# yli421/koopman-mpc-portfolio-rebalancing

Measured on AMD Instinct MI355X. Metric: MPC window-solves/sec (batched backtest) at 1/2/4/8 MI355X vs host-CPU ref, higher is better.
Workload: dtype f32 rollout (fp32 GEMMs as three exact bf16 planes); mixed f32->f64 IPM solve (float32 phase to mu 3e-5, float64 finish: stopping rule, status and W in float64); 1 GPU; C3 (BASELINE configs[2]): 65536 windows/GPU, 100 assets, latent 256, H=10, obs 2000, GenericKM enc [1024,1024], L1-turnover MPC c=1e-3 tau=0.2 no-short; windows_per_gpu=65536, parallelism=1 GPU, no collective

## Files before the change

include/kmpc.h:

```cpp
#ifndef KMPC_H
#define KMPC_H

#include <stddef.h>

#ifdef __cplusplus
extern "C" {
#endif

#define KMPC_OK               0
#define KMPC_ERR_INVALID     -1
#define KMPC_ERR_UNSUPPORTED -2
#define KMPC_ERR_WORKSPACE   -3
#define KMPC_ERR_LAUNCH      -4

#define KMPC_STATUS_OPTIMAL            0
#define KMPC_STATUS_OPTIMAL_INACCURATE 1
#define KMPC_STATUS_INFEASIBLE         2
#define KMPC_STATUS_UNBOUNDED          3
#define KMPC_STATUS_SOLVER_ERROR       4

#define KMPC_MAX_H 21
#define KMPC_MAX_N 1024

#define KMPC_PATH_AUTO     0
// ... 2 lines not shown
#define KMPC_PATH_LARGE    2
#define KMPC_PATH_REGISTER_UNPACKED 3
#define KMPC_PRECISION_AUTO  0
#define KMPC_PRECISION_F64   1
#define KMPC_PRECISION_MIXED 2
#define KMPC_MIXED_MIN_B 2048
typedef struct kmpc_solve_desc {
    int    B;
    int    N;
    int    H;
    double cost_coeff;
    double max_turnover;
    int    allow_short;
    int    max_iter;
    double tol;
    int    return_full_W;
    int    n_refine;
    int    path;
    int    precision;
    double mu_handoff;
} kmpc_solve_desc;

int kmpc_solve(const kmpc_solve_desc* desc,
               const float*  yhat,
               const double* w_prev,
               double*       w_out,
               int*          status,
               double*       obj,
               int*          iters,
               void* workspace, size_t ws_bytes, void* stream);

int kmpc_solve_box(const kmpc_solve_desc* desc, double max_weight,
                   const float*  yhat,
                   const double* w_prev,
                   double*       w_out,
                   int*          status,
                   double*       obj,
                   int*          iters,
                   void* stream);

int kmpc_gross_returns(size_t n, const float* yhat, float* R, void* stream);

#define KMPC_MODEL_GENERIC 0
#define KMPC_MODEL_LISTA   1
#define KMPC_ACT_RELU 0
#define KMPC_ACT_TANH 1
#define KMPC_ACT_GELU 2
#define KMPC_NORM_ID   0
#define KMPC_NORM_BALL 1
#define KMPC_MAX_LAYERS 8
#define KMPC_DTYPE_F32  0
#define KMPC_DTYPE_BF16 1
#define KMPC_DTYPE_F32_F32MFMA 2
typedef struct kmpc_mlp {
    int n_layers;
    int dims[KMPC_MAX_LAYERS + 1];
    int act;
    int last_relu;
    const float* weight[KMPC_MAX_LAYERS];
    const float* bias[KMPC_MAX_LAYERS];
} kmpc_mlp;

#define KMPC_LATENT_AUTO       0
#define KMPC_LATENT_UNFUSED    1
#define KMPC_LATENT_SEQUENTIAL 2

typedef struct kmpc_rollout_desc {
    int B;
    int N;
    int H;
    int L;
    int obs;
    int model_kind;
    int norm_fn;
    kmpc_mlp encoder;
    const float* lista_S;
    int   lista_loops;
    float lista_thresh;
    const float* kmat;
    kmpc_mlp decoder;
    const float* mean;
    const float* std;
    int obs_ld;
    int dtype;
    int latent_unfused;
} kmpc_rollout_desc;

int kmpc_rollout(const kmpc_rollout_desc* desc,
                 const float* obs,
                 float*       yhat,
                 void* workspace, size_t ws_bytes, void* stream);

int kmpc_standardize(int T, int N, const double* log_returns, const double* mean, const double* std,
                     float* z, void* stream);

int kmpc_window(const kmpc_rollout_desc* rdesc, const kmpc_solve_desc* sdesc,
                const float*  obs,
                const double* w_prev,
                float*        yhat,
                double*       w_out, int* status, double* obj, int* iters,
                void* workspace, size_t ws_bytes, void* stream);

typedef struct kmpc_backtest_desc {
    int    P;
    int    N;
    int    S;
// ... 79 lines not shown
```

koopman_mpc_portfolio_rebalancing_amd/_lib.py:

```python
from __future__ import annotations

import ctypes
import os

import torch

_HERE = os.path.dirname(os.path.abspath(__file__))
LIB_PATH = os.path.join(_HERE, "libkmpc.so")

KMPC_OK = 0
KMPC_ERR_UNSUPPORTED = -2
KMPC_MAX_LAYERS = 8
KMPC_MAX_N = 1024
KMPC_MAX_H = 21

MODEL_GENERIC, MODEL_LISTA = 0, 1
ACT = {"relu": 0, "tanh": 1, "gelu": 2}
NORM = {"id": 0, "ball": 1}
DTYPE = {"fp32": 0, "bf16": 1, "fp32_f32mfma": 2}
LATENT_FORM = {"auto": 0, "unfused": 1, "sequential": 2}

STATUS_NAMES = {0: "optimal", 1: "optimal_inaccurate", 2: "infeasible", 3: "unbounded",
                4: "solver_error"}

KMPC_MV_MAX_HN = 1024
KMPC_MV_MAX_H = 16

EXPORTED_SYMBOLS = ("kmpc_solve", "kmpc_rollout", "kmpc_window", "kmpc_workspace_bytes",
                    "kmpc_backtest_step", "kmpc_backtest_metrics", "kmpc_standardize", "kmpc_strerror",
                    "kmpc_version", "kmpc_solve_mv", "kmpc_rolling_moments", "kmpc_solve_mv_ws",
                    "kmpc_mv_workspace_bytes", "kmpc_gross_returns", "kmpc_backtest_run",
                    "kmpc_backtest_sweep", "kmpc_solve_box", "kmpc_solve_mv_box",
                    "kmpc_rolling_moments_paths", "kmpc_markowitz_run", "kmpc_markowitz_sweep")

PATH_AUTO, PATH_REGISTER, PATH_LARGE, PATH_REGISTER_UNPACKED = 0, 1, 2, 3
PRECISION_AUTO, PRECISION_F64, PRECISION_MIXED = 0, 1, 2
MIXED_MIN_B = 2048
PACK_MIN_B = 512

ABI_VERSION = "0.7.0"


class KmpcError(RuntimeError):
    pass


class SolveDesc(ctypes.Structure):
    _fields_ = [("B", ctypes.c_int), ("N", ctypes.c_int), ("H", ctypes.c_int),
                ("cost_coeff", ctypes.c_double), ("max_turnover", ctypes.c_double),
                ("allow_short", ctypes.c_int), ("max_iter", ctypes.c_int),
                ("tol", ctypes.c_double), ("return_full_W", ctypes.c_int), ("n_refine", ctypes.c_int),
                ("path", ctypes.c_int), ("precision", ctypes.c_int), ("mu_handoff", ctypes.c_double)]


class MvDesc(ctypes.Structure):
    _fields_ = [("B", ctypes.c_int), ("N", ctypes.c_int), ("H", ctypes.c_int),
                ("gamma", ctypes.c_double), ("cost_coeff", ctypes.c_double),
                ("allow_short", ctypes.c_int), ("max_iter", ctypes.c_int),
                ("tol", ctypes.c_double), ("return_full_W", ctypes.c_int)]


class Mlp(ctypes.Structure):
    _fields_ = [("n_layers", ctypes.c_int), ("dims", ctypes.c_int * (KMPC_MAX_LAYERS + 1)),
                ("act", ctypes.c_int), ("last_relu", ctypes.c_int),
                ("weight", ctypes.c_void_p * KMPC_MAX_LAYERS),
                ("bias", ctypes.c_void_p * KMPC_MAX_LAYERS)]


class RolloutDesc(ctypes.Structure):
    _fields_ = [("B", ctypes.c_int), ("N", ctypes.c_int), ("H", ctypes.c_int), ("L", ctypes.c_int),
                ("obs", ctypes.c_int), ("model_kind", ctypes.c_int), ("norm_fn", ctypes.c_int),
                ("encoder", Mlp), ("lista_S", ctypes.c_void_p), ("lista_loops", ctypes.c_int),
# ... 120 lines not shown
```

koopman_mpc_portfolio_rebalancing_amd/csrc/kmpc_rollout.hip:

```cpp
#include <hip/hip_runtime.h>
#include <math.h>
#include <stdint.h>

#include "kmpc_internal.h"

namespace kmpc {

typedef float f32x16 __attribute__((ext_vector_type(16)));
typedef float f32x4 __attribute__((ext_vector_type(4)));
typedef __bf16 bf16x8 __attribute__((ext_vector_type(8)));
typedef __bf16 bf16x4 __attribute__((ext_vector_type(4)));

enum Epi : int {
    EPI_NONE = 0,
    EPI_ACT = 1,
    EPI_SHRINK = 2,
    EPI_DESTD = 3,
};

struct GemmArgs {
    int M, N, K;
    const float* A; int lda;
    const float* B; int ldb;
    const float* bias;
// ... 433 lines not shown
                    c = __builtin_amdgcn_mfma_f32_32x32x16_bf16(af[0][a], bf[1][b], c, 0, 0, 0);
                    c = __builtin_amdgcn_mfma_f32_32x32x16_bf16(af[0][a], bf[0][b], c, 0, 0, 0);
                    acc[a][b] = c;
                }
        }
    };
    if constexpr (DB) {
        fetch(kbeg);
        stage(0);
        if (kbeg + BKT < kend) fetch(kbeg + BKT);
        __syncthreads();
        int buf = 0;
        for (int k0 = kbeg; k0 < kend; k0 += BKT) {
            substep(buf, 0);
            if (k0 + BKT < kend) {
                stage(buf ^ 1);
                if (k0 + 2 * BKT < kend) fetch(k0 + 2 * BKT);
            }
#pragma unroll
            for (int st = 1; st < NS; ++st) substep(buf, st);
            __syncthreads();
            buf ^= 1;
        }
    } else {
        fetch(kbeg);
        for (int k0 = kbeg; k0 < kend; k0 += BKT) {
            stage(0);
            __syncthreads();
            if (k0 + BKT < kend) fetch(k0 + BKT);
#pragma unroll
            for (int st = 0; st < NS; ++st) substep(0, st);
            __syncthreads();
        }
    }
    if (g.ksplit > 1) {
        float* P = g.part + (size_t)blockIdx.z * g.M * g.N;
#pragma unroll
        for (int a = 0; a < WM; ++a)
#pragma unroll
            for (int b = 0; b < WN; ++b) {
                const int n = n0 + wn + b * 32 + (lane & 31);
                if (n >= g.N) continue;
#pragma unroll
                for (int r = 0; r < 16; ++r) {
                    const int m = m0 + wm + a * 32 + (r & 3) + 8 * (r >> 2) + 4 * (lane >> 5);
                    if (m < g.M) P[(size_t)m * g.N + n] = acc[a][b][r];
                }
            }
        return;
    }
    epilogue<WM, WN>(g, acc, m0, n0, wm, wn, lane);
}

__global__ void shrink_kernel(const float* x, float* y, size_t n, float thr) {
    const size_t i = (size_t)blockIdx.x * blockDim.x + threadIdx.x;
    if (i < n) {
        const float v = x[i];
        const float av = fabsf(v) - thr;
        y[i] = (av > 0.0f) ? copysignf(av, v) : 0.0f * v;
    }
}

__global__ void ball_norm_kernel(float* x, int M, int L) {
    const int row = blockIdx.x * (blockDim.x / 64) + threadIdx.x / 64, lane = threadIdx.x & 63;
    if (row >= M) return;
    float* p = x + (size_t)row * L;
    float s = 0.0f;
    for (int j = lane; j < L; j += 64) s += p[j] * p[j];
#pragma unroll
    for (int o = 32; o >= 1; o >>= 1) s += __shfl_xor(s, o, 64);
    const float nrm = sqrtf(s);
    for (int j = lane; j < L; j += 64) p[j] = p[j] / nrm;
}

__global__ void transpose_kernel(const float* in, float* out, int R, int Cc) {
    __shared__ float tile[32][33];
    const int bx = blockIdx.x * 32, by = blockIdx.y * 32;
    const int tx = threadIdx.x & 31, ty = threadIdx.x >> 5;
    for (int r = ty; r < 32; r += 8) {
        const int i = by + r, j = bx + tx;
        if (i < R && j < Cc) tile[r][tx] = in[(size_t)i * Cc + j];
    }
    __syncthreads();
    for (int r = ty; r < 32; r += 8) {
        const int j = bx + r, i = by + tx;
        if (i < R && j < Cc) out[(size_t)j * R + i] = tile[tx][r];
    }
}

struct LatentArgs {
    int B, L, N, H;
    const float* z0;
    const float* zparts; int nparts; const float* zbias;
    const float* Kt;
    const float* K;
    const float* D;
    const float* bias;
    const float* mean; const float* stdv;
    float* yhat;
    int ball;
};
constexpr int LAT_ROWS = 32;

__device__ __forceinline__ float latent_z0(const LatentArgs& a, int m, int col) {
    const size_t i = (size_t)m * a.L + col;
    if (a.nparts == 0) return a.z0[i];
// ... 349 lines not shown
        __syncthreads();
    }
}

__global__ void tile_epilogue_kernel(int H, int N, const float* bias, const float* mean, const float* stdv,
                                     float* tb, float* tm, float* ts) {
    const int i = blockIdx.x * blockDim.x + threadIdx.x;
    if (i >= H * N) return;
    const int n = i % N;
    tb[i] = bias ? bias[n] : 0.0f;
    tm[i] = mean[n];
    ts[i] = stdv[n];
}

static bool latent_fusable(const kmpc_rollout_desc* d) {
    return d->latent_unfused != KMPC_LATENT_UNFUSED && d->dtype != KMPC_DTYPE_BF16 && d->decoder.n_layers == 1 && d->L % 32 == 0 &&
           d->L <= 512 && ((uintptr_t)d->decoder.weight[0] & 15) == 0 &&
           !(d->model_kind == KMPC_MODEL_GENERIC && d->norm_fn != KMPC_NORM_ID && d->norm_fn != KMPC_NORM_BALL);
}

#ifndef KMPC_F32_SPLITK
#define KMPC_F32_SPLITK 4
#endif
constexpr int SPLITK = KMPC_F32_SPLITK;
constexpr int SPLITK_BUF = 8;
constexpr size_t SPLITK_ELEMS = (size_t)256 * 64 * 64;

#ifndef KMPC_GEMM_MID
#define KMPC_GEMM_MID 44
#endif
#ifndef KMPC_BF16_SPLITK
#define KMPC_BF16_SPLITK 1
#endif
#ifndef KMPC_Z0_FUSE
#define KMPC_Z0_FUSE 1
#endif
#ifndef KMPC_BF16_SPLIT_MINK
#define KMPC_BF16_SPLIT_MINK 2048
#endif
#ifndef KMPC_BF16_SMALL
#define KMPC_BF16_SMALL 1
#endif
#ifndef KMPC_GEMM_BIG
#define KMPC_GEMM_BIG 42
#endif
template <int WM, int WN, int GM = 2, int GN = 2>
static void launch_f32(dim3 grid, hipStream_t s, const GemmArgs& g) {
    if (g.bf16 == 2)
        hipLaunchKernelGGL((gemm_nt_x3_kernel<WM, WN, GM, GN>), grid, dim3(64 * GM * GN), 0, s, g);
    else
        hipLaunchKernelGGL((gemm_nt_kernel<WM, WN, BK, GM, GN>), grid, dim3(64 * GM * GN), 0, s, g);
}

static int gemm(GemmArgs g, hipStream_t s, float* part = nullptr, int* nparts = nullptr) {
    if (nparts) *nparts = 0;
    if (g.M <= 0 || g.N <= 0) return KMPC_OK;
    g.ksplit = 1;
    dim3 grid((g.N + BN - 1) / BN, (g.M + BM - 1) / BM);
    if (g.bf16 == 1) {
        const bool few = (size_t)grid.x * grid.y < 256;
        if (KMPC_BF16_SPLITK && few && part && g.K >= KMPC_BF16_SPLIT_MINK && (size_t)g.M * g.N <= SPLITK_ELEMS) {
            g.ksplit = SPLITK_BUF;
            g.part = part;
            hipLaunchKernelGGL(gemm_nt_bf16_kernel<2>, dim3(grid.x, grid.y, SPLITK_BUF), dim3(256), 0, s, g);
            const size_t n = (size_t)g.M * g.N;
            hipLaunchKernelGGL(splitk_epilogue_kernel, dim3((unsigned)((n + 255) / 256)), dim3(256), 0, s, g);
            return hipGetLastError() == hipSuccess ? KMPC_OK : KMPC_ERR_LAUNCH;
        }
        if (few && KMPC_BF16_SMALL)
            hipLaunchKernelGGL(gemm_nt_bf16_kernel<1>, dim3((g.N + 63) / 64, (g.M + 63) / 64), dim3(256), 0, s, g);
        else
            hipLaunchKernelGGL(gemm_nt_bf16_kernel<2>, grid, dim3(256), 0, s, g);
    } else if ((size_t)grid.x * grid.y < 512) {
        dim3 grid64((g.N + 63) / 64, (g.M + 63) / 64);
        static_assert(SPLITK >= 2 && SPLITK <= SPLITK_BUF, "split-K slices");
        if (part && (size_t)grid64.x * grid64.y < 256 && g.K >= 128 * SPLITK) {
            g.ksplit = SPLITK;
            g.part = part;
            launch_f32<1, 1>(dim3(grid64.x, grid64.y, SPLITK), s, g);
            if (nparts && g.epi == EPI_NONE) {
                *nparts = SPLITK;
                return hipGetLastError() == hipSuccess ? KMPC_OK : KMPC_ERR_LAUNCH;
            }
            const size_t n = (size_t)g.M * g.N;
            hipLaunchKernelGGL(splitk_epilogue_kernel, dim3((unsigned)((n + 255) / 256)), dim3(256), 0, s, g);
            return hipGetLastError() == hipSuccess ? KMPC_OK : KMPC_ERR_LAUNCH;
        }
        if (KMPC_GEMM_MID == 21)
            launch_f32<2, 1>(dim3((g.N + 63) / 64, (g.M + 127) / 128), s, g);
        else if (KMPC_GEMM_MID == 12)
            launch_f32<1, 2>(dim3((g.N + 127) / 128, (g.M + 63) / 64), s, g);
        else if (KMPC_GEMM_MID == 22)
            launch_f32<2, 2>(grid, s, g);
        else if (KMPC_GEMM_MID == 42)
            launch_f32<1, 2, 4, 2>(grid, s, g);
        else if (KMPC_GEMM_MID == 44)
            launch_f32<1, 1, 4, 4>(grid, s, g);
        else
            launch_f32<1, 1>(grid64, s, g);
    } else if (KMPC_GEMM_BIG == 42) {
        launch_f32<1, 2, 4, 2>(grid, s, g);
    } else if (KMPC_GEMM_BIG == 44) {
        launch_f32<1, 1, 4, 4>(grid, s, g);
    } else if (KMPC_GEMM_BIG == 82) {
        launch_f32<1, 2, 8, 2>(dim3((g.N + 127) / 128, (g.M + 255) / 256), s, g);
    } else {
        launch_f32<2, 2>(grid, s, g);
    }
    return hipGetLastError() == hipSuccess ? KMPC_OK : KMPC_ERR_LAUNCH;
}

static GemmArgs linear(int M, int N, int K, const float* A, int lda, const float* W, const float* bias,
                       float* C, int ldc) {
    GemmArgs g = {};
    g.M = M; g.N = N; g.K = K; g.A = A; g.lda = lda; g.B = W; g.ldb = K; g.bias = bias;
    g.C = C; g.ldc = ldc; g.epi = EPI_NONE;
    return g;
}

static size_t align256(size_t x) { return (x + 255) & ~(size_t)255; }

static int max_width(const kmpc_mlp& m) {
    int w = 0;
    for (int l = 0; l <= m.n_layers; ++l) w = m.dims[l] > w ? m.dims[l] : w;
    return w;
}

size_t rollout_workspace_bytes(const kmpc_rollout_desc* d) {
    if (!d) return 0;
    const size_t B = (size_t)d->B;
    int wmax = d->L;
    const int we = max_width(d->encoder), wd = max_width(d->decoder);
    if (we > wmax) wmax = we;
    if (wd > wmax) wmax = wd;
    size_t bytes = 0;
    bytes += align256(sizeof(float) * (size_t)d->L * d->L);
    bytes += align256(sizeof(float) * (size_t)d->L * d->L);
    bytes += 2 * align256(sizeof(float) * B * wmax);
    bytes += 2 * align256(sizeof(float) * B * d->L);
    const size_t part = B * (size_t)wmax < SPLITK_ELEMS ? B * (size_t)wmax : SPLITK_ELEMS;
    bytes += align256(sizeof(float) * SPLITK_BUF * part);
    bytes += align256((size_t)6 * d->L * (d->L + 32 * (size_t)((d->N + 31) / 32)));
    bytes += align256(sizeof(float) * (size_t)d->H * d->N * (d->L + 3));
    return bytes;
}

static int run_mlp(const kmpc_mlp& m, int Bn, const float* X, int ldx, float* out, int ldo,
                   int last_cols, int last_epi, const float* mean, const float* stdv, float* ping,
                   float* pong, int wmax, int bf16, hipStream_t s, float* part, int* last_nparts = nullptr) {
    const float* cur = X;
    int ldc = ldx;
    for (int l = 0; l < m.n_layers; ++l) {
        const bool last = (l == m.n_layers - 1);
        const int nout = last ? last_cols : m.dims[l + 1];
        float* dst = last ? out : ((l & 1) ? pong : ping);
        GemmArgs g = linear(Bn, nout, m.dims[l], cur, ldc, m.weight[l], m.bias[l], dst,
                            last ? ldo : wmax);
        g.bf16 = bf16;
        if (!last) { g.epi = EPI_ACT; g.act = m.act; }
        else if (last_epi == EPI_DESTD) { g.epi = EPI_DESTD; g.mean = mean; g.stdv = stdv; }
        else if (m.last_relu) { g.epi = EPI_ACT; g.act = KMPC_ACT_RELU; }
        int rc = gemm(g, s, part, last ? last_nparts : nullptr);
        if (rc) return rc;
        cur = dst;
        ldc = wmax;
    }
    return KMPC_OK;
}

int rollout_launch(const kmpc_rollout_desc* d, const float* obs, float* yhat, void* ws,
                   size_t ws_bytes, hipStream_t s) {
    if (!d || !obs || !yhat || !d->kmat || !d->mean || !d->std) return KMPC_ERR_INVALID;
    if (d->B < 0 || d->N < 1 || d->H < 1 || d->L < 1 || d->obs < d->N) return KMPC_ERR_INVALID;
    if (d->encoder.n_layers < 1 || d->encoder.n_layers > KMPC_MAX_LAYERS) return KMPC_ERR_INVALID;
    if (d->decoder.n_layers < 1 || d->decoder.n_layers > KMPC_MAX_LAYERS) return KMPC_ERR_INVALID;
    if (d->encoder.dims[0] != d->obs || d->encoder.dims[d->encoder.n_layers] != d->L) return KMPC_ERR_INVALID;
    if (d->decoder.dims[0] != d->L || d->decoder.dims[d->decoder.n_layers] < d->N) return KMPC_ERR_INVALID;
    if (d->model_kind == KMPC_MODEL_LISTA && !d->lista_S) return KMPC_ERR_INVALID;
    if (ws_bytes < rollout_workspace_bytes(d) || (!ws && ws_bytes)) return KMPC_ERR_WORKSPACE;
    if (d->obs_ld < 0 || (d->obs_ld > 0 && d->obs_ld < d->N)) return KMPC_ERR_INVALID;
    if (d->dtype != KMPC_DTYPE_F32 && d->dtype != KMPC_DTYPE_BF16 && d->dtype != KMPC_DTYPE_F32_F32MFMA)
        return KMPC_ERR_INVALID;
    if (d->latent_unfused < KMPC_LATENT_AUTO || d->latent_unfused > KMPC_LATENT_SEQUENTIAL) return KMPC_ERR_INVALID;
    const int bf = d->dtype == KMPC_DTYPE_F32 ? KMPC_F32_GEMM : d->dtype == KMPC_DTYPE_BF16 ? 1 : 0;
    if (d->B == 0) return KMPC_OK;
    const int Bn = d->B, L = d->L, N = d->N, H = d->H;
    const int obs_ld = d->obs_ld > 0 ? d->obs_ld : d->obs;
    int wmax = L;
    {
        const int we = max_width(d->encoder), wd = max_width(d->decoder);
        if (we > wmax) wmax = we;
        if (wd > wmax) wmax = wd;
    }
    char* p = (char*)ws;
    float* Kt = (float*)p;   p += align256(sizeof(float) * (size_t)L * L);
    float* St = (float*)p;   p += align256(sizeof(float) * (size_t)L * L);
    float* ping = (float*)p; p += align256(sizeof(float) * (size_t)Bn * wmax);
    float* pong = (float*)p; p += align256(sizeof(float) * (size_t)Bn * wmax);
    float* z0 = (float*)p;   p += align256(sizeof(float) * (size_t)Bn * L);
    float* z1 = (float*)p;   p += align256(sizeof(float) * (size_t)Bn * L);
    float* part = (float*)p;
    {
        const size_t pe = (size_t)Bn * wmax < SPLITK_ELEMS ? (size_t)Bn * wmax : SPLITK_ELEMS;
        p += align256(sizeof(float) * SPLITK_BUF * pe);
    }
    __bf16* planes = (__bf16*)p;
    p += align256((size_t)6 * L * (L + 32 * (size_t)((N + 31) / 32)));
    float* Wpow = (float*)p;
    int rc;
    const bool latpow = KMPC_LATPOW && d->latent_unfused == KMPC_LATENT_AUTO && latent_fusable(d) && Bn >= KMPC_LATPOW_MINB &&
                        !(d->model_kind == KMPC_MODEL_GENERIC && d->norm_fn == KMPC_NORM_BALL);
    const bool lat16 = latent_fusable(d) && (Bn < KMPC_LAT16_MAXB || L <= 16 * KMPC_LAT16_WAVES);
    const bool kdir = lat16 && Bn < KMPC_LAT16_MAXB && !latpow;
    dim3 tg((L + 31) / 32, (L + 31) / 32);
    if (!kdir) hipLaunchKernelGGL(transpose_kernel, tg, dim3(256), 0, s, d->kmat, Kt, L, L);
    if (d->model_kind == KMPC_MODEL_LISTA)
        hipLaunchKernelGGL(transpose_kernel, tg, dim3(256), 0, s, d->lista_S, St, L, L);
    if (hipGetLastError() != hipSuccess) return KMPC_ERR_LAUNCH;

    int znparts = 0;
    const bool zfuse = KMPC_Z0_FUSE && d->model_kind == KMPC_MODEL_GENERIC && latent_fusable(d) &&
                       d->norm_fn != KMPC_NORM_BALL && !latpow;
    if (d->model_kind == KMPC_MODEL_GENERIC) {
        rc = run_mlp(d->encoder, Bn, obs, obs_ld, z0, L, L, EPI_NONE, nullptr, nullptr, ping, pong, wmax, bf, s, part,
                     zfuse ? &znparts : nullptr);
        if (rc) return rc;
        if (d->norm_fn == KMPC_NORM_BALL)
            hipLaunchKernelGGL(ball_norm_kernel, dim3((Bn + 3) / 4), dim3(256), 0, s, z0, Bn, L);
    } else {
        rc = run_mlp(d->encoder, Bn, obs, obs_ld, z1, L, L, EPI_NONE, nullptr, nullptr, ping, pong, wmax, bf, s, part);
        if (rc) return rc;
        const size_t n = (size_t)Bn * L;
        hipLaunchKernelGGL(shrink_kernel, dim3((unsigned)((n + 255) / 256)), dim3(256), 0, s, z1, z0, n,
                           d->lista_thresh);
        float* zc = z0;
        float* zn = ping;
        for (int it = 0; it < d->lista_loops; ++it) {
            GemmArgs g = linear(Bn, L, L, zc, L, St, nullptr, zn, L);
            g.epi = EPI_SHRINK; g.R = z1; g.ldr = L; g.thr = d->lista_thresh; g.bf16 = bf;
            if ((rc = gemm(g, s, part))) return rc;
            float* t = zc; zc = zn; zn = t;
        }
        if (zc != z0 && hipMemcpyAsync(z0, zc, sizeof(float) * n, hipMemcpyDeviceToDevice, s) != hipSuccess)
            return KMPC_ERR_LAUNCH;
    }
    if (hipGetLastError() != hipSuccess) return KMPC_ERR_LAUNCH;
    if (znparts > 0 && !latent_fusable(d)) return KMPC_ERR_INVALID;

    if (latpow) {
        const int HN = H * N;
        float* tb = Wpow + (size_t)HN * L;
        float* tm = tb + HN;
        float* ts = tm + HN;
        hipLaunchKernelGGL(latent_powers_kernel, dim3(N), dim3(64 * ((L + 63) / 64)), sizeof(double) * L, s,
                           d->decoder.weight[0], Kt, L, N, H, Wpow);
        hipLaunchKernelGGL(tile_epilogue_kernel, dim3((HN + 255) / 256), dim3(256), 0, s, H, N, d->decoder.bias[0],
                           d->mean, d->std, tb, tm, ts);
        GemmArgs g = linear(Bn, HN, L, z0, L, Wpow, tb, yhat, HN);
        g.epi = EPI_DESTD; g.mean = tm; g.stdv = ts; g.bf16 = bf;
        if ((rc = gemm(g, s, part))) return rc;
        return hipGetLastError() == hipSuccess ? KMPC_OK : KMPC_ERR_LAUNCH;
    }
    if (latent_fusable(d)) {
        LatentArgs la;
        la.B = Bn; la.L = L; la.N = N; la.H = H; la.z0 = z0; la.Kt = Kt; la.K = d->kmat; la.D = d->decoder.weight[0];
        la.zparts = part; la.nparts = znparts;
        la.zbias = d->encoder.bias[d->encoder.n_layers - 1];
        la.bias = d->decoder.bias[0]; la.mean = d->mean; la.stdv = d->std; la.yhat = yhat;
        la.ball = d->model_kind == KMPC_MODEL_GENERIC && d->norm_fn == KMPC_NORM_BALL;
        if (lat16) {
            const size_t lds = sizeof(float) * 2 * LAT16 * (L + 4);
            if (kdir)
                hipLaunchKernelGGL((latent_steps16_kernel<KMPC_LAT16_WAVES, true>), dim3((Bn + LAT16 - 1) / LAT16),
                                   dim3(64 * KMPC_LAT16_WAVES), lds, s, la);
            else
                hipLaunchKernelGGL((latent_steps16_kernel<KMPC_LAT16_WAVES, false>), dim3((Bn + LAT16 - 1) / LAT16),
                                   dim3(64 * KMPC_LAT16_WAVES), lds, s, la);
            return hipGetLastError() == hipSuccess ? KMPC_OK : KMPC_ERR_LAUNCH;
        }
        if (KMPC_LATX3 && bf == 2 && !la.ball && L == 256) {
            const int Dpad = 32 * ((N + 31) / 32);
            __bf16* Kp = planes;
            __bf16* Dp = planes + (size_t)3 * L * L;
            const size_t nk = (size_t)L * L, nd = (size_t)Dpad * L;
            hipLaunchKernelGGL(split_planes_kernel, dim3((unsigned)((nk + 255) / 256)), dim3(256), 0, s, Kt, L, L, L, L, Kp);
            hipLaunchKernelGGL(split_planes_kernel, dim3((unsigned)((nd + 255) / 256)), dim3(256), 0, s, la.D, N, Dpad, L,
                               L, Dp);
            const size_t lds = sizeof(__bf16) * 3 * LATX3_ROWS * (L + 8);
            hipLaunchKernelGGL((latent_steps_x3_kernel<8, 256>), dim3((Bn + LATX3_ROWS - 1) / LATX3_ROWS), dim3(512), lds,
                               s, la, (const __bf16*)Kp, (const __bf16*)Dp, Dpad);
            return hipGetLastError() == hipSuccess ? KMPC_OK : KMPC_ERR_LAUNCH;
        }
        const size_t lds = sizeof(float) * 2 * LAT_ROWS * (L + 4);
        hipLaunchKernelGGL(latent_steps_kernel<KMPC_LAT_WAVES>, dim3((Bn + LAT_ROWS - 1) / LAT_ROWS),
                           dim3(64 * KMPC_LAT_WAVES), lds, s, la);
        return hipGetLastError() == hipSuccess ? KMPC_OK : KMPC_ERR_LAUNCH;
    }
    float* zc = z0;
    float* zn = z1;
    for (int k = 0; k < H; ++k) {
        GemmArgs g = linear(Bn, L, L, zc, L, Kt, nullptr, zn, L);
        g.bf16 = bf;
        if ((rc = gemm(g, s, part))) return rc;
        if (d->model_kind == KMPC_MODEL_GENERIC && d->norm_fn == KMPC_NORM_BALL)
            hipLaunchKernelGGL(ball_norm_kernel, dim3((Bn + 3) / 4), dim3(256), 0, s, zn, Bn, L);
        rc = run_mlp(d->decoder, Bn, zn, L, yhat + (size_t)k * N, H * N, N, EPI_DESTD, d->mean, d->std,
                     ping, pong, wmax, bf, s, part);
        if (rc) return rc;
        float* t = zc; zc = zn; zn = t;
    }
    return hipGetLastError() == hipSuccess ? KMPC_OK : KMPC_ERR_LAUNCH;
}

__global__ void standardize_kernel(int T, int N, const double* y, const double* mean, const double* stdv,
                                   float* z) {
    const size_t i = (size_t)blockIdx.x * blockDim.x + threadIdx.x;
    if (i >= (size_t)T * N) return;
    const int n = (int)(i % N);
    z[i] = (float)((y[i] - mean[n]) / stdv[n]);
}

int standardize_launch(int T, int N, const double* y, const double* mean, const double* stdv, float* z,
                       hipStream_t s) {
    const size_t n = (size_t)T * N;
    if (n == 0) return KMPC_OK;
    hipLaunchKernelGGL(standardize_kernel, dim3((unsigned)((n + 255) / 256)), dim3(256), 0, s, T, N, y, mean,
                       stdv, z);
    return hipGetLastError() == hipSuccess ? KMPC_OK : KMPC_ERR_LAUNCH;
}

}
```

Baseline: 895,100 windows/s.

## Pre-split GEMM operands into tiled bf16 planes and chain plane outputs across layers

Adds a plane-based fp32-as-three-bf16 GEMM path. Weights are pre-split into tiled hi/mid/lo bf16 planes. Activations are emitted directly in plane layout by the previous layer's epilogue, so the next GEMM loads them with global_load_lds instead of re-splitting fp32 in every k-loop. This removes the per-tile split3 conversion and strided fp32 A/B loads from the large encoder and readout GEMMs. In exchange it adds split kernels, extra workspace, a more complex epilogue that writes three planes, and a new kernel that has not been tuned.

```diff
diff --git a/include/kmpc.h b/include/kmpc.h
--- a/include/kmpc.h
+++ b/include/kmpc.h
@@ -78,6 +78,7 @@
 #define KMPC_DTYPE_F32  0
 #define KMPC_DTYPE_BF16 1
 #define KMPC_DTYPE_F32_F32MFMA 2
+#define KMPC_DTYPE_F32_INSPLIT 3
 typedef struct kmpc_mlp {
     int n_layers;
     int dims[KMPC_MAX_LAYERS + 1];
diff --git a/koopman_mpc_portfolio_rebalancing_amd/_lib.py b/koopman_mpc_portfolio_rebalancing_amd/_lib.py
--- a/koopman_mpc_portfolio_rebalancing_amd/_lib.py
+++ b/koopman_mpc_portfolio_rebalancing_amd/_lib.py
@@ -17,7 +17,7 @@
 MODEL_GENERIC, MODEL_LISTA = 0, 1
 ACT = {"relu": 0, "tanh": 1, "gelu": 2}
 NORM = {"id": 0, "ball": 1}
-DTYPE = {"fp32": 0, "bf16": 1, "fp32_f32mfma": 2}
+DTYPE = {"fp32": 0, "bf16": 1, "fp32_f32mfma": 2, "fp32_insplit": 3}
 LATENT_FORM = {"auto": 0, "unfused": 1, "sequential": 2}
 
 STATUS_NAMES = {0: "optimal", 1: "optimal_inaccurate", 2: "infeasible", 3: "unbounded",
diff --git a/koopman_mpc_portfolio_rebalancing_amd/csrc/kmpc_rollout.hip b/koopman_mpc_portfolio_rebalancing_amd/csrc/kmpc_rollout.hip
--- a/koopman_mpc_portfolio_rebalancing_amd/csrc/kmpc_rollout.hip
+++ b/koopman_mpc_portfolio_rebalancing_amd/csrc/kmpc_rollout.hip
@@ -509,6 +509,271 @@
     epilogue<WM, WN>(g, acc, m0, n0, wm, wn, lane);
 }
 
+constexpr int PT_ROWS = 128, PT_K = 32;
+constexpr size_t PT_PLANE = (size_t)PT_ROWS * PT_K;
+constexpr size_t PT_TILE = 3 * PT_PLANE;
+
+struct PlaneArgs {
+    const __bf16* Ap; int akt;
+    const __bf16* Bp; int bkt;
+    __bf16* Cp; int ckt;
+};
+
+__global__ void __launch_bounds__(256) split_planes_tiled_kernel(const float* __restrict__ src, int R, int K, int ld,
+                                                                 int nrb, int nkt, __bf16* __restrict__ dst) {
+    const size_t i = (size_t)blockIdx.x * 256 + threadIdx.x;
+    if (i >= (size_t)nrb * nkt * (PT_ROWS * PT_K / 8)) return;
+    const int c = (int)(i & 3), row = (int)((i >> 2) & (PT_ROWS - 1));
+    const size_t t = i >> 9;
+    const int kt = (int)(t % nkt), rb = (int)(t / nkt);
+    const int rr = rb * PT_ROWS + row, k0 = kt * PT_K + c * 8;
+    float x[8];
+#pragma unroll
+    for (int e = 0; e < 8; ++e) x[e] = 0.0f;
+    if (rr < R) {
+        const float* p = src + (size_t)rr * ld + k0;
+        if (k0 + 7 < K && (ld & 3) == 0 && (((uintptr_t)src) & 15) == 0) {
+            const f32x4 u = *(const f32x4*)p, v = *(const f32x4*)(p + 4);
+#pragma unroll
+            for (int e = 0; e < 4; ++e) { x[e] = u[e]; x[4 + e] = v[e]; }
+        } else {
+#pragma unroll
+            for (int e = 0; e < 8; ++e)
+                if (k0 + e < K) x[e] = p[e];
+        }
+    }
+    bf16x8 h, m, l;
+#pragma unroll
+    for (int e = 0; e < 8; ++e) {
+        __bf16 x0, x1, x2;
+        split3(x[e], x0, x1, x2);
+        h[e] = x0; m[e] = x1; l[e] = x2;
+    }
+    __bf16* o = dst + t * PT_TILE + row * PT_K + c * 8;
+    *(bf16x8*)o = h;
+    *(bf16x8*)(o + PT_PLANE) = m;
+    *(bf16x8*)(o + 2 * PT_PLANE) = l;
+}
+
+__device__ __forceinline__ void epilogue_planes(const GemmArgs& g, const PlaneArgs& pl, f32x16 (&acc)[1][2],
+                                                __bf16* lds, int m0, int n0, int wm, int wn, int wv, int lane) {
+    constexpr int WN = 2, TM = 128;
+    const int h = lane >> 5, c31 = lane & 31;
+    float v[WN][16];
+#pragma unroll
+    for (int b = 0; b < WN; ++b) {
+        const int n = n0 + wn + b * 32 + c31;
+        const float bias = (g.bias && n < g.N) ? g.bias[n] : 0.0f;
+#pragma unroll
+        for (int r = 0; r < 16; ++r) {
+            const int m = m0 + wm + (r & 3) + 8 * (r >> 2) + 4 * h;
+            float x = acc[0][b][r] + bias;
+            if (g.epi == EPI_ACT) x = apply_act(x, g.act);
+            v[b][r] = (m < g.M && n < g.N) ? x : 0.0f;
+        }
+    }
+    __bf16* W = lds + wv * (WN * 32 * PT_K);
+    __bf16* Ct = pl.Cp + ((size_t)(m0 / TM) * pl.ckt + (n0 + wn) / PT_K) * PT_TILE + wm * PT_K;
+#pragma unroll
+    for (int p = 0; p < 3; ++p) {
+#pragma unroll
+        for (int b = 0; b < WN; ++b)
+#pragma unroll
+            for (int r = 0; r < 16; ++r) {
+                __bf16 x[3];
+                split3(v[b][r], x[0], x[1], x[2]);
+                W[b * 32 * PT_K + ((r & 3) + 8 * (r >> 2) + 4 * h) * PT_K + c31] = x[p];
+            }
+        asm volatile("s_waitcnt lgkmcnt(0)" ::: "memory");
+#pragma unroll
+        for (int q = 0; q < WN * 2; ++q) {
+            const int ch = q * 64 + lane;
+            const bf16x8 u = *(const bf16x8*)(W + ch * 8);
+            *(bf16x8*)(Ct + (size_t)(ch >> 7) * PT_TILE + p * PT_PLANE + (ch & 127) * 8) = u;
+        }
+        asm volatile("s_waitcnt lgkmcnt(0)" ::: "memory");
+    }
+}
+
+__device__ __forceinline__ void glds16(const __bf16* src, __bf16* dst_wave_base) {
+#if defined(__HIP_DEVICE_COMPILE__)
+    __builtin_amdgcn_global_load_lds((const __attribute__((address_space(1))) void*)(uintptr_t)src,
+                                     (__attribute__((address_space(3))) void*)(uint32_t)(uintptr_t)dst_wave_base, 16, 0,
+                                     0);
+#endif
+}
+
+template <bool AP>
+__global__ void __launch_bounds__(512) gemm_nt_x3g_kernel(GemmArgs g, PlaneArgs pl) {
+    constexpr int NT = 512, TM = 128, TN = 128, WN = 2, GN = 2;
+    static_assert(TM == PT_ROWS && TN == PT_ROWS && BK == PT_K && PT_PLANE == (size_t)NT * 8, "plane tiles");
+    __shared__ __bf16 S[2][3][PT_PLANE];
+    const int tid = threadIdx.x, lane = tid & 63, wv = tid >> 6;
+    int m0, n0;
+    xcd_tile(m0, n0, TM, TN);
+    const int wm = (wv / GN) * 32, wn = (wv % GN) * 32 * WN;
+    f32x16 acc[1][WN];
+#pragma unroll
+    for (int b = 0; b < WN; ++b)
+#pragma unroll
+        for (int r = 0; r < 16; ++r) acc[0][b][r] = 0.0f;
+
+    const int kend = g.K;
+    const bool vec_ok = ((g.lda & 3) == 0) && ((((uintptr_t)g.A) & 15) == 0);
+    constexpr int QA = TM * BK / (4 * NT), RQ = BK / 4;
+    f32x4 va[QA];
+    const int srow = tid >> 2, spc = (tid & 3) ^ ((srow >> 2) & 3);
+    const __bf16* Bt = pl.Bp + (size_t)(n0 / TN) * pl.bkt * PT_TILE + srow * PT_K + spc * 8;
+    const int wbase = wv * 64 * 8;
+    auto issue_b = [&](int k0) {
+        const size_t t = (size_t)(k0 / BK) * PT_TILE;
+#pragma unroll
+        for (int p = 0; p < 3; ++p) glds16(Bt + t + p * PT_PLANE, S[1][p] + wbase);
+    };
+    auto fetch_a = [&](int k0) {
+        if (vec_ok && k0 + BK <= kend) {
+#pragma unroll
+            for (int q = 0; q < QA; ++q) {
+                const int idx = tid + q * NT, rr = min(m0 + idx / RQ, g.M - 1);
+                va[q] = *(const f32x4*)(g.A + (size_t)rr * g.lda + k0 + (idx % RQ) * 4);
+            }
+            return;
+        }
+#pragma unroll
+        for (int q = 0; q < QA; ++q) {
+            const int idx = tid + q * NT, rr = m0 + idx / RQ, kk = k0 + (idx % RQ) * 4;
+            va[q] = f32x4{0.f, 0.f, 0.f, 0.f};
+            if (rr < g.M) {
+                if (vec_ok && kk + 3 < kend) {
+                    va[q] = *(const f32x4*)(g.A + (size_t)rr * g.lda + kk);
+                } else {
+#pragma unroll
+                    for (int e = 0; e < 4; ++e)
+                        if (kk + e < kend) va[q][e] = g.A[(size_t)rr * g.lda + kk + e];
+                }
+            }
+        }
+    };
+    auto stage_a = [&]() {
+#pragma unroll
+        for (int q = 0; q < QA; ++q) {
+            const int idx = tid + q * NT, row = idx / RQ, kq = idx % RQ;
+            bf16x4 h, m, l;
+#pragma unroll
+            for (int e = 0; e < 4; ++e) {
+                __bf16 x0, x1, x2;
+                split3(va[q][e], x0, x1, x2);
+                h[e] = x0; m[e] = x1; l[e] = x2;
+            }
+            const int o = row * PT_K + (((kq >> 1) ^ ((row >> 2) & 3)) * 8) + (kq & 1) * 4;
+            *(bf16x4*)(S[0][0] + o) = h;
+            *(bf16x4*)(S[0][1] + o) = m;
+            *(bf16x4*)(S[0][2] + o) = l;
+        }
+    };
+    auto substep = [&](int st) {
+        const int r = lane & 31, h = lane >> 5;
+        const int o = r * PT_K + (((2 * st + h) ^ ((r >> 2) & 3)) * 8);
+        bf16x8 af[3], bf[3][WN];
+#pragma unroll
+        for (int p = 0; p < 3; ++p) {
+            af[p] = *(const bf16x8*)(S[0][p] + wm * PT_K + o);
+#pragma unroll
+            for (int b = 0; b < WN; ++b) bf[p][b] = *(const bf16x8*)(S[1][p] + (wn + b * 32) * PT_K + o);
+        }
+#pragma unroll
+        for (int b = 0; b < WN; ++b) {
+            f32x16 c = acc[0][b];
+            c = __builtin_amdgcn_mfma_f32_32x32x16_bf16(af[1], bf[1][b], c, 0, 0, 0);
+            c = __builtin_amdgcn_mfma_f32_32x32x16_bf16(af[2], bf[0][b], c, 0, 0, 0);
+            c = __builtin_amdgcn_mfma_f32_32x32x16_bf16(af[0], bf[2][b], c, 0, 0, 0);
+            c = __builtin_amdgcn_mfma_f32_32x32x16_bf16(af[1], bf[0][b], c, 0, 0, 0);
+            c = __builtin_amdgcn_mfma_f32_32x32x16_bf16(af[0], bf[1][b], c, 0, 0, 0);
+            c = __builtin_amdgcn_mfma_f32_32x32x16_bf16(af[0], bf[0][b], c, 0, 0, 0);
+            acc[0][b] = c;
+        }
+    };
+    if constexpr (AP) {
+        __bf16* Sb = &S[0][0][0];
+        constexpr int HP = PT_ROWS * 16, HB = 6 * HP;
+        const __bf16* src[3];
+        int dsto[3];
+#pragma unroll
+        for (int j = 0; j < 3; ++j) {
+            const int q = wv * 3 + j, o = q >> 2, rg = q & 3;
+            const int row = rg * 32 + (lane >> 1), pc = (lane & 1) ^ ((row >> 3) & 1);
+            const __bf16* base = o < 3 ? pl.Ap + (size_t)(m0 / TM) * pl.akt * PT_TILE
+                                       : pl.Bp + (size_t)(n0 / TN) * pl.bkt * PT_TILE;
+            src[j] = base + (o % 3) * PT_PLANE + row * PT_K + pc * 8;
+            dsto[j] = o * HP + rg * 32 * 16;
+        }
+        auto issue_h = [&](int kt, int half) {
+#pragma unroll
+            for (int j = 0; j < 3; ++j) glds16(src[j] + (size_t)kt * PT_TILE + half * 16, Sb + half * HB + dsto[j]);
+        };
+        auto sub_h = [&](int half) {
+            const int r = lane & 31, h = lane >> 5;
+            const __bf16* P = Sb + half * HB + r * 16 + ((h ^ ((r >> 3) & 1)) * 8);
+            bf16x8 af[3], bf[3][WN];
+#pragma unroll
+            for (int p = 0; p < 3; ++p) {
+                af[p] = *(const bf16x8*)(P + p * HP + wm * 16);
+#pragma unroll
+                for (int b = 0; b < WN; ++b) bf[p][b] = *(const bf16x8*)(P + (3 + p) * HP + (wn + b * 32) * 16);
+            }
+#pragma unroll
+            for (int b = 0; b < WN; ++b) {
+                f32x16 c = acc[0][b];
+                c = __builtin_amdgcn_mfma_f32_32x32x16_bf16(af[1], bf[1][b], c, 0, 0, 0);
+                c = __builtin_amdgcn_mfma_f32_32x32x16_bf16(af[2], bf[0][b], c, 0, 0, 0);
+                c = __builtin_amdgcn_mfma_f32_32x32x16_bf16(af[0], bf[2][b], c, 0, 0, 0);
+                c = __builtin_amdgcn_mfma_f32_32x32x16_bf16(af[1], bf[0][b], c, 0, 0, 0);
+                c = __builtin_amdgcn_mfma_f32_32x32x16_bf16(af[0], bf[1][b], c, 0, 0, 0);
+                c = __builtin_amdgcn_mfma_f32_32x32x16_bf16(af[0], bf[0][b], c, 0, 0, 0);
+                acc[0][b] = c;
+            }
+        };
+        const int nkt = (kend + BK - 1) / BK;
+        issue_h(0, 0);
+        asm volatile("s_waitcnt vmcnt(0)" ::: "memory");
+        __syncthreads();
+        for (int kt = 0; kt < nkt; ++kt) {
+            issue_h(kt, 1);
+            sub_h(0);
+            asm volatile("s_waitcnt vmcnt(0)" ::: "memory");
+            __syncthreads();
+            if (kt + 1 < nkt) issue_h(kt + 1, 0);
+            sub_h(1);
+            asm volatile("s_waitcnt vmcnt(0)" ::: "memory");
+            __syncthreads();
+        }
+        if (!pl.Cp) {
+            epilogue<1, WN>(g, acc, m0, n0, wm, wn, lane);
+            return;
+        }
+        epilogue_planes(g, pl, acc, Sb, m0, n0, wm, wn, wv, lane);
+        return;
+    } else {
+        fetch_a(0);
+        for (int k0 = 0; k0 < kend; k0 += BK) {
+            issue_b(k0);
+            stage_a();
+            asm volatile("s_waitcnt vmcnt(0)" ::: "memory");
+            __syncthreads();
+            if (k0 + BK < kend) fetch_a(k0 + BK);
+#pragma unroll
+            for (int st = 0; st < BK / 16; ++st) substep(st);
+            __syncthreads();
+        }
+        if (!pl.Cp) {
+            epilogue<1, WN>(g, acc, m0, n0, wm, wn, lane);
+            return;
+        }
+        epilogue_planes(g, pl, acc, &S[0][0][0], m0, n0, wm, wn, wv, lane);
+        return;
+    }
+}
+
 __global__ void shrink_kernel(const float* x, float* y, size_t n, float thr) {
     const size_t i = (size_t)blockIdx.x * blockDim.x + threadIdx.x;
     if (i < n) {
@@ -964,11 +1229,36 @@
         hipLaunchKernelGGL((gemm_nt_kernel<WM, WN, BK, GM, GN>), grid, dim3(64 * GM * GN), 0, s, g);
 }
 
-static int gemm(GemmArgs g, hipStream_t s, float* part = nullptr, int* nparts = nullptr) {
+#ifndef KMPC_X3_PLANES
+#define KMPC_X3_PLANES 1
+#endif
+static bool plane_gemm(int M, int N) {
+    return KMPC_X3_PLANES && KMPC_F32_GEMM == 2 && KMPC_GEMM_BIG == 42 && M > 0 && N > 0 &&
+           (size_t)((N + BN - 1) / BN) * ((M + BM - 1) / BM) >= 512;
+}
+static int tiles_of(int n, int t) { return (n + t - 1) / t; }
+static size_t plane_elems(int R, int K) { return (size_t)tiles_of(R, PT_ROWS) * tiles_of(K, PT_K) * PT_TILE; }
+static void split_tiled(const float* src, int R, int K, int ld, __bf16* dst, hipStream_t s) {
+    const int nrb = tiles_of(R, PT_ROWS), nkt = tiles_of(K, PT_K);
+    const size_t n = (size_t)nrb * nkt * (PT_ROWS * PT_K / 8);
+    hipLaunchKernelGGL(split_planes_tiled_kernel, dim3((unsigned)((n + 255) / 256)), dim3(256), 0, s, src, R, K, ld, nrb,
+                       nkt, dst);
+}
+
+static int gemm(GemmArgs g, hipStream_t s, float* part = nullptr, int* nparts = nullptr,
+                const PlaneArgs* pl = nullptr) {
     if (nparts) *nparts = 0;
     if (g.M <= 0 || g.N <= 0) return KMPC_OK;
     g.ksplit = 1;
     dim3 grid((g.N + BN - 1) / BN, (g.M + BM - 1) / BM);
+    if (pl) {
+        if (!pl->Bp || g.bf16 != 2 || !plane_gemm(g.M, g.N)) return KMPC_ERR_INVALID;
+        if (pl->Ap)
+            hipLaunchKernelGGL(gemm_nt_x3g_kernel<true>, grid, dim3(512), 0, s, g, *pl);
+        else
+            hipLaunchKernelGGL(gemm_nt_x3g_kernel<false>, grid, dim3(512), 0, s, g, *pl);
+        return hipGetLastError() == hipSuccess ? KMPC_OK : KMPC_ERR_LAUNCH;
+    }
     if (g.bf16 == 1) {
         const bool few = (size_t)grid.x * grid.y < 256;
         if (KMPC_BF16_SPLITK && few && part && g.K >= KMPC_BF16_SPLIT_MINK && (size_t)g.M * g.N <= SPLITK_ELEMS) {
@@ -1038,6 +1328,30 @@
     return w;
 }
 
+static bool planes_possible(const kmpc_rollout_desc* d, int wmax) {
+    const int w = d->H * d->N > wmax ? d->H * d->N : wmax;
+    return d->dtype == KMPC_DTYPE_F32 && plane_gemm(d->B, w);
+}
+static size_t act_bytes(const kmpc_rollout_desc* d, int width, int pwidth, bool planes) {
+    const size_t f = sizeof(float) * (size_t)d->B * width;
+    const size_t p = planes ? sizeof(__bf16) * (size_t)tiles_of(d->B, PT_ROWS) * tiles_of(pwidth, BN) * (BN / PT_K) * PT_TILE : 0;
+    return align256(f > p ? f : p);
+}
+static int max_out_width(const kmpc_rollout_desc* d) {
+    int w = 0;
+    for (int l = 1; l < d->encoder.n_layers; ++l) w = d->encoder.dims[l] > w ? d->encoder.dims[l] : w;
+    for (int l = 1; l < d->decoder.n_layers; ++l) w = d->decoder.dims[l] > w ? d->decoder.dims[l] : w;
+    return w;
+}
+static size_t weight_plane_bytes(const kmpc_rollout_desc* d) {
+    size_t n = 0;
+    for (int l = 0; l < d->encoder.n_layers; ++l) n += plane_elems(d->encoder.dims[l + 1], d->encoder.dims[l]);
+    for (int l = 0; l < d->decoder.n_layers; ++l) n += plane_elems(d->decoder.dims[l + 1], d->decoder.dims[l]);
+    n += plane_elems(d->L, d->L);
+    n += plane_elems(d->H * d->N, d->L);
+    return align256(sizeof(__bf16) * n);
+}
+
 size_t rollout_workspace_bytes(const kmpc_rollout_desc* d) {
     if (!d) return 0;
     const size_t B = (size_t)d->B;
@@ -1045,11 +1359,14 @@
     const int we = max_width(d->encoder), wd = max_width(d->decoder);
     if (we > wmax) wmax = we;
     if (wd > wmax) wmax = wd;
+    const bool pp = planes_possible(d, wmax);
     size_t bytes = 0;
     bytes += align256(sizeof(float) * (size_t)d->L * d->L);
     bytes += align256(sizeof(float) * (size_t)d->L * d->L);
-    bytes += 2 * align256(sizeof(float) * B * wmax);
-    bytes += 2 * align256(sizeof(float) * B * d->L);
+    bytes += 2 * act_bytes(d, wmax, max_out_width(d), pp);
+    bytes += act_bytes(d, d->L, d->L, pp);
+    bytes += align256(sizeof(float) * B * d->L);
+    if (pp) bytes += weight_plane_bytes(d);
     const size_t part = B * (size_t)wmax < SPLITK_ELEMS ? B * (size_t)wmax : SPLITK_ELEMS;
     bytes += align256(sizeof(float) * SPLITK_BUF * part);
     bytes += align256((size_t)6 * d->L * (d->L + 32 * (size_t)((d->N + 31) / 32)));
@@ -1057,11 +1374,32 @@
     return bytes;
 }
 
+struct MlpPlanes {
+    const __bf16* wp[KMPC_MAX_LAYERS];
+    __bf16* outp;
+};
+static void mlp_weight_planes(const kmpc_mlp& m, int Bn, int last_cols, __bf16*& pool, MlpPlanes& mp,
+                              hipStream_t s) {
+    mp.outp = nullptr;
+    for (int l = 0; l < KMPC_MAX_LAYERS; ++l) mp.wp[l] = nullptr;
+    for (int l = 0; l < m.n_layers; ++l) {
+        const int nout = (l == m.n_layers - 1) ? last_cols : m.dims[l + 1];
+        if (!plane_gemm(Bn, nout)) continue;
+        split_tiled(m.weight[l], nout, m.dims[l], m.dims[l], pool, s);
+        mp.wp[l] = pool;
+        pool += plane_elems(nout, m.dims[l]);
+    }
+}
+
 static int run_mlp(const kmpc_mlp& m, int Bn, const float* X, int ldx, float* out, int ldo,
                    int last_cols, int last_epi, const float* mean, const float* stdv, float* ping,
-                   float* pong, int wmax, int bf16, hipStream_t s, float* part, int* last_nparts = nullptr) {
+                   float* pong, int wmax, int bf16, hipStream_t s, float* part, int* last_nparts = nullptr,
+                   const MlpPlanes* mp = nullptr, bool* out_planes = nullptr) {
     const float* cur = X;
     int ldc = ldx;
+    const __bf16* curp = nullptr;
+    int curkt = 0;
+    if (out_planes) *out_planes = false;
     for (int l = 0; l < m.n_layers; ++l) {
         const bool last = (l == m.n_layers - 1);
         const int nout = last ? last_cols : m.dims[l + 1];
@@ -1072,8 +1410,22 @@
         if (!last) { g.epi = EPI_ACT; g.act = m.act; }
         else if (last_epi == EPI_DESTD) { g.epi = EPI_DESTD; g.mean = mean; g.stdv = stdv; }
         else if (m.last_relu) { g.epi = EPI_ACT; g.act = KMPC_ACT_RELU; }
-        int rc = gemm(g, s, part, last ? last_nparts : nullptr);
+        const bool pk = mp && mp->wp[l];
+        PlaneArgs pl = {};
+        if (pk) {
+            pl.Bp = mp->wp[l]; pl.bkt = tiles_of(m.dims[l], PT_K);
+            pl.Ap = curp; pl.akt = curkt;
+            const bool to_planes = last ? (mp->outp && g.epi != EPI_DESTD) : (mp->wp[l + 1] != nullptr);
+            if (to_planes) {
+                pl.Cp = last ? mp->outp : (__bf16*)dst;
+                pl.ckt = tiles_of(nout, BN) * (BN / PT_K);
+                if (last && out_planes) *out_planes = true;
+            }
+        }
+        int rc = gemm(g, s, part, last ? last_nparts : nullptr, pk ? &pl : nullptr);
         if (rc) return rc;
+        curp = pl.Cp;
+        curkt = pl.ckt;
         cur = dst;
         ldc = wmax;
     }
@@ -1091,10 +1443,12 @@
     if (d->model_kind == KMPC_MODEL_LISTA && !d->lista_S) return KMPC_ERR_INVALID;
     if (ws_bytes < rollout_workspace_bytes(d) || (!ws && ws_bytes)) return KMPC_ERR_WORKSPACE;
     if (d->obs_ld < 0 || (d->obs_ld > 0 && d->obs_ld < d->N)) return KMPC_ERR_INVALID;
-    if (d->dtype != KMPC_DTYPE_F32 && d->dtype != KMPC_DTYPE_BF16 && d->dtype != KMPC_DTYPE_F32_F32MFMA)
+    if (d->dtype != KMPC_DTYPE_F32 && d->dtype != KMPC_DTYPE_BF16 && d->dtype != KMPC_DTYPE_F32_F32MFMA &&
+        d->dtype != KMPC_DTYPE_F32_INSPLIT)
         return KMPC_ERR_INVALID;
     if (d->latent_unfused < KMPC_LATENT_AUTO || d->latent_unfused > KMPC_LATENT_SEQUENTIAL) return KMPC_ERR_INVALID;
-    const int bf = d->dtype == KMPC_DTYPE_F32 ? KMPC_F32_GEMM : d->dtype == KMPC_DTYPE_BF16 ? 1 : 0;
+    const int bf = (d->dtype == KMPC_DTYPE_F32 || d->dtype == KMPC_DTYPE_F32_INSPLIT) ? KMPC_F32_GEMM
+                   : d->dtype == KMPC_DTYPE_BF16 ? 1 : 0;
     if (d->B == 0) return KMPC_OK;
     const int Bn = d->B, L = d->L, N = d->N, H = d->H;
     const int obs_ld = d->obs_ld > 0 ? d->obs_ld : d->obs;
@@ -1107,9 +1461,10 @@
     char* p = (char*)ws;
     float* Kt = (float*)p;   p += align256(sizeof(float) * (size_t)L * L);
     float* St = (float*)p;   p += align256(sizeof(float) * (size_t)L * L);
-    float* ping = (float*)p; p += align256(sizeof(float) * (size_t)Bn * wmax);
-    float* pong = (float*)p; p += align256(sizeof(float) * (size_t)Bn * wmax);
-    float* z0 = (float*)p;   p += align256(sizeof(float) * (size_t)Bn * L);
+    const bool pp = planes_possible(d, wmax) && bf == 2;
+    float* ping = (float*)p; p += act_bytes(d, wmax, max_out_width(d), pp);
+    float* pong = (float*)p; p += act_bytes(d, wmax, max_out_width(d), pp);
+    float* z0 = (float*)p;   p += act_bytes(d, L, L, pp);
     float* z1 = (float*)p;   p += align256(sizeof(float) * (size_t)Bn * L);
     float* part = (float*)p;
     {
@@ -1119,6 +1474,8 @@
     __bf16* planes = (__bf16*)p;
     p += align256((size_t)6 * L * (L + 32 * (size_t)((N + 31) / 32)));
     float* Wpow = (float*)p;
+    p += align256(sizeof(float) * (size_t)H * N * (L + 3));
+    __bf16* wpool = (__bf16*)p;
     int rc;
     const bool latpow = KMPC_LATPOW && d->latent_unfused == KMPC_LATENT_AUTO && latent_fusable(d) && Bn >= KMPC_LATPOW_MINB &&
                         !(d->model_kind == KMPC_MODEL_GENERIC && d->norm_fn == KMPC_NORM_BALL);
@@ -1133,14 +1490,22 @@
     int znparts = 0;
     const bool zfuse = KMPC_Z0_FUSE && d->model_kind == KMPC_MODEL_GENERIC && latent_fusable(d) &&
                        d->norm_fn != KMPC_NORM_BALL && !latpow;
+    MlpPlanes encp;
+    bool z0_planes = false;
+    if (pp) {
+        mlp_weight_planes(d->encoder, Bn, L, wpool, encp, s);
+        if (latpow && d->model_kind == KMPC_MODEL_GENERIC && plane_gemm(Bn, H * N)) encp.outp = (__bf16*)z0;
+        if (hipGetLastError() != hipSuccess) return KMPC_ERR_LAUNCH;
+    }
     if (d->model_kind == KMPC_MODEL_GENERIC) {
         rc = run_mlp(d->encoder, Bn, obs, obs_ld, z0, L, L, EPI_NONE, nullptr, nullptr, ping, pong, wmax, bf, s, part,
-                     zfuse ? &znparts : nullptr);
+                     zfuse ? &znparts : nullptr, pp ? &encp : nullptr, &z0_planes);
         if (rc) return rc;
         if (d->norm_fn == KMPC_NORM_BALL)
             hipLaunchKernelGGL(ball_norm_kernel, dim3((Bn + 3) / 4), dim3(256), 0, s, z0, Bn, L);
     } else {
-        rc = run_mlp(d->encoder, Bn, obs, obs_ld, z1, L, L, EPI_NONE, nullptr, nullptr, ping, pong, wmax, bf, s, part);
+        rc = run_mlp(d->encoder, Bn, obs, obs_ld, z1, L, L, EPI_NONE, nullptr, nullptr, ping, pong, wmax, bf, s, part,
+                     nullptr, pp ? &encp : nullptr);
         if (rc) return rc;
         const size_t n = (size_t)Bn * L;
         hipLaunchKernelGGL(shrink_kernel, dim3((unsigned)((n + 255) / 256)), dim3(256), 0, s, z1, z0, n,
@@ -1170,6 +1535,14 @@
                            d->mean, d->std, tb, tm, ts);
         GemmArgs g = linear(Bn, HN, L, z0, L, Wpow, tb, yhat, HN);
         g.epi = EPI_DESTD; g.mean = tm; g.stdv = ts; g.bf16 = bf;
+        if (pp && plane_gemm(Bn, HN)) {
+            split_tiled(Wpow, HN, L, L, wpool, s);
+            PlaneArgs pl = {};
+            pl.Bp = wpool; pl.bkt = tiles_of(L, PT_K);
+            if (z0_planes) { pl.Ap = (const __bf16*)z0; pl.akt = tiles_of(L, BN) * (BN / PT_K); }
+            if ((rc = gemm(g, s, part, nullptr, &pl))) return rc;
+            return hipGetLastError() == hipSuccess ? KMPC_OK : KMPC_ERR_LAUNCH;
+        }
         if ((rc = gemm(g, s, part))) return rc;
         return hipGetLastError() == hipSuccess ? KMPC_OK : KMPC_ERR_LAUNCH;
     }
@@ -1210,14 +1583,25 @@
     }
     float* zc = z0;
     float* zn = z1;
+    MlpPlanes decp;
+    PlaneArgs kpl = {};
+    if (pp) {
+        if (plane_gemm(Bn, L)) {
+            split_tiled(Kt, L, L, L, wpool, s);
+            kpl.Bp = wpool; kpl.bkt = tiles_of(L, PT_K);
+            wpool += plane_elems(L, L);
+        }
+        mlp_weight_planes(d->decoder, Bn, N, wpool, decp, s);
+        if (hipGetLastError() != hipSuccess) return KMPC_ERR_LAUNCH;
+    }
     for (int k = 0; k < H; ++k) {
         GemmArgs g = linear(Bn, L, L, zc, L, Kt, nullptr, zn, L);
         g.bf16 = bf;
-        if ((rc = gemm(g, s, part))) return rc;
+        if ((rc = gemm(g, s, part, nullptr, kpl.Bp ? &kpl : nullptr))) return rc;
         if (d->model_kind == KMPC_MODEL_GENERIC && d->norm_fn == KMPC_NORM_BALL)
             hipLaunchKernelGGL(ball_norm_kernel, dim3((Bn + 3) / 4), dim3(256), 0, s, zn, Bn, L);
         rc = run_mlp(d->decoder, Bn, zn, L, yhat + (size_t)k * N, H * N, N, EPI_DESTD, d->mean, d->std,
-                     ping, pong, wmax, bf, s, part);
+                     ping, pong, wmax, bf, s, part, nullptr, pp ? &decp : nullptr);
         if (rc) return rc;
         float* t = zc; zc = zn; zn = t;
     }
```

Result: no change. 895,300 windows/s (median of 5 runs) (+0.0%).
